# RKlompUU/fhe-regex

Measured on AMD Instinct MI355X. Metric: TFHE gate-bootstraps/sec; end-to-end match time for /abc/ on 256-char content, higher is better.
Workload: dtype u64

## Files before the change

fhe-regex_amd/csrc/capi.cpp:

```cpp
#include <climits>
#include <cstring>
#include <string>
#include <vector>

#include "ctx.h"
#include "rns.h"

using namespace fr;

namespace fr {

static thread_local std::string g_last_error;
void set_last_error(const std::string& m) { g_last_error = m; }

Params params_from_c(const fr_params* c) {
    Params p;
    if (c) {
        p.k = c->k;
        p.N = c->N;
        p.n = c->n;
        p.ks_base_log = c->ks_base_log;
        p.ks_level = c->ks_level;
        p.pbs_base_log = c->pbs_base_log;
        p.pbs_level = c->pbs_level;
        p.ring = c->ring;
        p.lwe_sigma = c->lwe_sigma;
        p.glwe_sigma = c->glwe_sigma;
    }
    validate_params(p);
    return p;
}
void validate_params(const Params& p) {
    if (p.k < 1 || p.k > 4 || p.N < 256 || p.N > 4096 || (p.N & (p.N - 1)) || p.n < 1 || p.n > 1024)
        throw Error(FR_ERR_INVALID, "invalid params");
    if (p.pbs_base_log != 23 || p.pbs_level != 1) throw Error(FR_ERR_INVALID, "only the 2^23 x 1 PBS gadget is supported");
    if (p.ks_base_log < 1 || p.ks_base_log * p.ks_level > 63) throw Error(FR_ERR_INVALID, "invalid keyswitch gadget");
    if (p.ring != FR_RING_RNS && p.ring != FR_RING_FFT) throw Error(FR_ERR_INVALID, "invalid ring");
    if (p.ring == FR_RING_FFT && !((p.k == 1 && p.N == 2048) || (p.k == 2 && p.N == 1024)))
        throw Error(FR_ERR_INVALID, "the FFT ring is built for (k, N) = (1, 2048) and (2, 1024)");
}

}

static Program one_output(std::vector<PGate>&& gates) {
    Program p;
    p.gates = std::move(gates);
    p.outs.push_back(ProgOut{(int32_t)p.gates.size() - 1, 1, 0});
    compute_levels(p);
    return p;
}
static Program prog_cmp_const(VNode::Op op, uint8_t c) {
    const bool sign = op != VNode::EQ;
    return one_output({nibble_test_gate(sign, 0, 0, c & 15), nibble_test_gate(sign, 0, 1, c >> 4), cmp_final_gate(op, 0, 1)});
}

extern "C" {

const char* fr_last_error(void) { return fr::g_last_error.c_str(); }

int fr_default_params(fr_params* out) {
    FR_TRY({
        NEED(out);
        Params p;
        std::memset(out, 0, sizeof *out);
        out->k = p.k;
        out->N = p.N;
        out->n = p.n;
        out->ks_base_log = p.ks_base_log;
        out->ks_level = p.ks_level;
        out->pbs_base_log = p.pbs_base_log;
        out->pbs_level = p.pbs_level;
        out->ring = p.ring;
        out->lwe_sigma = p.lwe_sigma;
        out->glwe_sigma = p.glwe_sigma;
    })
}

int fr_ctx_create(const fr_params* params, int device, fr_ctx** out) {
    FR_TRY({
        NEED(out);
        *out = nullptr;
        auto ctx = std::make_unique<fr_ctx>();
        ctx->p = params_from_c(params);
        if (device >= 0) ctx->dev = std::make_unique<Device>(ctx->p, device);
        *out = ctx.release();
    })
}

int fr_ctx_destroy(fr_ctx* ctx) {
// ... 462 lines not shown
        NEED((content || !len) && tables && any && start_lo <= start_hi && (starts_out || start_lo == start_hi));
        NEED(m >= 1 && m <= NEEDLE_MAX_CHARS);
        plain_needle(MATCH_NEEDLE_CLEAR, content, len, len, m, start_lo, start_hi, nullptr, nullptr, starts_out, any,
                     tables);
    })
}
int fr_plain_scan_clear_bytes(const uint8_t* content, size_t len, const uint8_t* tables, size_t m, size_t start_lo,
                              size_t start_hi, uint8_t* starts_out, int32_t* any) {
    FR_TRY({
        NEED((content || !len) && tables && any && start_lo <= start_hi && (starts_out || start_lo == start_hi));
        NEED(m >= 1 && m <= NEEDLE_MAX_CHARS && start_hi - start_lo <= ((size_t)1 << 24));
        WindowClasses wc = window_classes(content, len, m, start_lo, start_hi);
        pad_window_text(wc, m);
        plain_needle(MATCH_NEEDLE_WINDOWS, wc.text.data(), wc.text.size(), scan_padded(wc.first.size()), m, start_lo,
                     start_hi, nullptr, &wc.cls, starts_out, any, tables);
    })
}
int fr_dev_select_sum(fr_ctx* ctx, const fr_needle* needle, const uint8_t* content, size_t len, const int32_t* terms,
                      const int32_t* n_terms, size_t n_sums, uint64_t* out) {
    FR_TRY({
        NEED(ctx && needle && (content || !len) && terms && n_terms && out);
        Device& dev = ctx->device();
        if (needle->k != ctx->p.k || needle->N != ctx->p.N)
            throw Error(FR_ERR_INVALID, "needle: k, N do not match the context params");
        dev.select_sum_host(needle->dev, content, len, terms, n_terms, n_sums, out);
    })
}
int fr_dev_select_sum_ms(fr_ctx* ctx, double* ms) {
    FR_TRY({
        NEED(ctx && ms);
        *ms = ctx->device().select_sum_ms();
    })
}
int fr_dev_ring_mul(fr_ctx* ctx, const uint64_t* a, const uint64_t* b, size_t count, uint64_t* out) {
    FR_TRY({
        NEED(ctx && a && b && out);
        ctx->device().ring_mul_host(a, b, count, out);
    })
}
int fr_dev_bench_pbs(fr_ctx* ctx, const fr_ct* in, size_t count, int32_t iters, double* br_ms, double* total_ms) {
    FR_TRY({
        NEED(ctx && in && count && iters > 0 && br_ms && total_ms);
        Device& dev = ctx->device();
        if (!ctx->has_sk) throw Error(FR_ERR_NO_KEY, "server key not generated");
        std::vector<DevGate> gates(count);
        for (size_t i = 0; i < count; ++i) {
            const HandleRec& h = ctx->get(in[i]);
            DevGate& d = gates[i];
            std::memset(&d, 0, sizeof d);
            int nin = 0, off = 0;
            const int w[2] = {1, 4};
            for (int b = 0; b < (h.is_bool ? 1 : 2); ++b) {
                if (h.b[b].slot < 0) {
                    off += w[b] * h.b[b].triv;
                    continue;
                }
                d.in_slot[nin] = h.b[b].slot;
                d.in_w[nin] = w[b];
                ++nin;
            }
            d.n_in = nin;
            d.offset = 2 * off;
            lut_eq(d.lut[0], 1);
            d.n_out = 1;
            d.direct = JOB_DIRECT;
        }
        Slots outs(dev, count);
        for (size_t i = 0; i < count; ++i) gates[i].out_slot[0] = outs[i];
        dev.bench_pbs(gates, iters, br_ms, total_ms);
    })
}

uint64_t fr_debug_scalar(int32_t op, uint64_t x, uint64_t y) {
    switch (op) {
        case 0: return rns::crt((uint32_t)(x % rns::P0), (uint32_t)(x % rns::P1));
        case 1: return (uint64_t)(int64_t)rns::decompose((uint32_t)(x % rns::P0), (uint32_t)(x % rns::P1));
        case 2: return rns::to_torus((uint32_t)(x % rns::P0), (uint32_t)(x % rns::P1));
        case 3: return mod_switch(x, (int)y);
        case 4: {
            int32_t d[5];
            ks_decompose<3, 5>(x, d);
            return (uint64_t)(int64_t)d[y % 5];
        }
        default: return 0;
    }
}

int fr_debug_arena_stats(fr_ctx* ctx, uint64_t* slots, uint64_t* free_slots) {
    FR_TRY({
        NEED(ctx && slots && free_slots);
        Device& dev = ctx->device();
        dev.sync();
        *slots = dev.arena_slots();
        *free_slots = dev.arena_free_slots();
    })
}

int fr_debug_handle_count(fr_ctx* ctx, uint64_t* live) {
    FR_TRY({
        NEED(ctx && live);
        *live = ctx->handles.size() - ctx->free_handles.size();
    })
}

int fr_export_bool_device(fr_ctx* ctx, const fr_ct* h, size_t n, uint64_t* dev_dst) {
    FR_TRY({
        NEED(ctx && (h || !n) && (dev_dst || !n));
        Device& dev = ctx->device();
        std::vector<int> slots(n);
        size_t n_triv = 0;
        for (size_t i = 0; i < n; ++i) {
            slots[i] = ctx->get(h[i]).b[0].slot;
            n_triv += slots[i] < 0;
        }
        Slots tmp(dev, n_triv);
        std::vector<uint64_t> lwe((size_t)ctx->p.lwe_len(), 0);
        for (size_t i = 0, t = 0; i < n; ++i) {
            if (slots[i] >= 0) continue;
            lwe.back() = (uint64_t)ctx->get(h[i]).b[0].triv << DELTA_LOG;
            slots[i] = tmp[t++];
            dev.write_slots(&slots[i], 1, lwe.data());
        }
        dev.slots_to_device(slots.data(), n, dev_dst);
    })
}
int fr_export_bool_device_async(fr_ctx* ctx, const fr_ct* h, size_t n, uint64_t* dev_dst) {
    FR_TRY({
        NEED(ctx && (h || !n) && (dev_dst || !n));
        if (n > 16) throw Error(FR_ERR_INVALID, "fr_export_bool_device_async: at most 16 handles");
        std::vector<int> slots(n);
        for (size_t i = 0; i < n; ++i) {
            const HandleRec& r = ctx->get(h[i]);
            if (r.b[0].slot < 0) return fr_export_bool_device(ctx, h, n, dev_dst);
            slots[i] = r.b[0].slot;
        }
        ctx->device().slots_to_device_async(slots.data(), n, dev_dst);
    })
}
int fr_stream(fr_ctx* ctx, void** stream) {
    FR_TRY({
        NEED(ctx && stream);
        *stream = ctx->device().stream();
    })
}
int fr_import_bool_device(fr_ctx* ctx, const uint64_t* dev_src, size_t n, fr_ct* out) {
    FR_TRY({
        NEED(ctx && out && (dev_src || !n));
        Device& dev = ctx->device();
        Slots slots(dev, n);
        dev.device_to_slots(slots.data(), n, dev_src);
        ctx->adopt(std::move(slots), false, out);
    })
}
static int device_timers(fr_ctx* ctx, double DeviceTimers::*ms, uint64_t DeviceTimers::*launches,
                         uint64_t DeviceTimers::*gates, double* br_ms, double* ks_ms, uint64_t* br_launches,
                         uint64_t* br_gates) {
    FR_TRY({
        NEED(ctx);
        Device& dev = ctx->device();
        dev.sync();
        const DeviceTimers& t = dev.timers();
        if (br_ms) *br_ms = t.*ms;
        if (ks_ms) *ks_ms = t.ks_ms;
        if (br_launches) *br_launches = t.*launches;
        if (br_gates) *br_gates = t.*gates;
    })
// ... 34 lines not shown
```

fhe-regex_amd/csrc/fft_br.hip:

```cpp
#include <hip/hip_ext.h>
#include <hip/hip_runtime.h>

#include <cstring>

#include "device_impl.h"
#include "fft.h"
#include "geo.h"

namespace fr {

template <int M, int E>
using FGeo = NttGeo<M, E, 3, fft_layout_variant(ilog2c(M), ilog2c(E))>;
template <int M, int E>
constexpr int FV = fft_layout_variant(ilog2c(M), ilog2c(E));

__device__ __forceinline__ void cfwd(double2& x, double2& y, double2 c) { fft::fwd_bf(x.x, x.y, y.x, y.y, c.x, c.y); }
__device__ __forceinline__ void cinv(double2& u, double2& v, double2 c) { fft::inv_bf(u.x, u.y, v.x, v.y, c.x, c.y); }

template <int M, int E>
constexpr bool fradix4() {
    return E == 4 && FGeo<M, E>::LOG % 2 == 0;
}
template <int M, int E>
struct FTwr {
    static constexpr int COUNT = fradix4<M, E>() ? FGeo<M, E>::NPH * 3 : FGeo<M, E>::LOG * (E / 2);
    double2 v[COUNT];
};
__device__ __forceinline__ double2 fmul_i(double2 c) { return make_double2(-c.y, c.x); }
__device__ __forceinline__ void cinv_r4(double2 (&x)[4], double2 c, double2 ca, double2 cc) {
    fft::inv_r4(x[0].x, x[0].y, x[1].x, x[1].y, x[2].x, x[2].y, x[3].x, x[3].y, c.x, c.y, ca.x, ca.y, cc.x, cc.y);
}
template <class G, int E, int p, bool REV, class F>
__device__ __forceinline__ void for_butterflies(F&& fn) {
#pragma unroll
    for (int i = 0; i < G::s_end(p) - G::s_begin(p); ++i) {
        const int s = REV ? G::s_end(p) - 1 - i : G::s_begin(p) + i;
        const int dm = 1 << (G::LOG - 1 - s - G::lo(p));
#pragma unroll
        for (int m = 0; m < E; ++m) {
            if (m & dm) continue;
            fn(s, m, dm);
        }
    }
}
template <class G, int p>
__device__ __forceinline__ double2 ftw_at(const double2* tw, int b, int s, int m) {
    return (tw + (b >> (G::LOG - s)))[(1 << s) + (G::template moff<p>(m) >> (G::LOG - s))];
}
template <int M, int E, int p>
__device__ __forceinline__ void ftw_r4(const double2* tw, int tl, double2& c, double2& ca) {
    using G = FGeo<M, E>;
    constexpr int s0 = G::s_begin(p), s1 = s0 + 1;
    const int b = G::template base<p>(tl);
    c = ftw_at<G, p>(tw, b, s0, 0);
    ca = ftw_at<G, p>(tw, b, s1, 0);
}

template <int M, int E, int p>
__device__ __forceinline__ void ffwd_phase(double2 (&x)[E], const double2* tw, int tl) {
    using G = FGeo<M, E>;
    const int b = G::template base<p>(tl);
    for_butterflies<G, E, p, false>([&](int s, int m, int dm) { cfwd(x[m], x[m + dm], ftw_at<G, p>(tw, b, s, m)); });
}
template <int M, int E, int p>
__device__ __forceinline__ void finv_phase(double2 (&x)[E], const double2* tw, int tl) {
    using G = FGeo<M, E>;
    const int b = G::template base<p>(tl);
    for_butterflies<G, E, p, true>([&](int s, int m, int dm) { cinv(x[m], x[m + dm], ftw_at<G, p>(tw, b, s, m)); });
}
template <int M, int E, int p>
__device__ __forceinline__ void finv_phase_lds(double2 (&x)[E], const double2* tw, const double2* twc, int tl) {
    if constexpr (fradix4<M, E>()) {
        using G = FGeo<M, E>;
        double2 c, ca;
        ftw_r4<M, E, p>(tw, tl, c, ca);
        const double2 cc = ftw_at<G, p>(twc, G::template base<p>(tl), G::s_begin(p), 0);
        cinv_r4(x, c, ca, cc);
    } else {
        finv_phase<M, E, p>(x, tw, tl);
    }
}

template <int M, int E, int p>
constexpr bool ftw_wave_uniform() {
    using G = FGeo<M, E>;
    for (int w = 0; w * 64 < G::T; ++w)
        for (int s = G::s_begin(p); s < G::s_end(p); ++s) {
            const int ref = geo_base(G::LOG, G::e, p, w * 64, FV<M, E>) >> (G::LOG - s);
            for (int l = 1; l < 64; ++l)
                if ((geo_base(G::LOG, G::e, p, w * 64 + l, FV<M, E>) >> (G::LOG - s)) != ref) return false;
// ... 235 lines not shown
template <int K, int NB, class KeyAt>
__device__ __forceinline__ void key_products(const double (&bre)[2][NB], const double (&bim)[2][NB], int mb, uint32_t ei,
                                             uint32_t ej, uint32_t sm, KeyAt&& key, double& kor, double& koi,
                                             double (&kxr)[K], double (&kxi)[K]) {
    double cr[3], ci[3];
#pragma unroll
    for (int h = 1; h < 3; ++h)
        slot_factor(bre[h - 1][mb], bim[h - 1][mb], h == 1 ? ei : ej, sm, cr[h], ci[h]);
    fft::cmul(cr[1], ci[1], cr[2], ci[2], cr[0], ci[0]);
#pragma unroll
    for (int gg = 0; gg < 3; ++gg) {
        const double c1r = cr[gg] - 1.0, c1i = ci[gg];
        const double2 Bo = key(gg, 0);
        if (gg == 0) fft::cmul(Bo.x, Bo.y, c1r, c1i, kor, koi);
        else fft::cmac(Bo.x, Bo.y, c1r, c1i, kor, koi);
#pragma unroll
        for (int q = 0; q < K; ++q) {
            const double2 Bx = key(gg, 1 + q);
            if (gg == 0) fft::cmul(Bx.x, Bx.y, c1r, c1i, kxr[q], kxi[q]);
            else fft::cmac(Bx.x, Bx.y, c1r, c1i, kxr[q], kxi[q]);
        }
    }
}
constexpr int KEY_AHEAD = -1;
constexpr int KEY_TOP = -2;
constexpr int KEY_NEVER = -3;
struct FbrKeySchedule {
    int g[3];
    constexpr int group_at(int when) const {
        for (int i = 0; i < 3; ++i)
            if (g[i] == when) return i;
        return 3;
    }
    constexpr int ahead() const { return (g[0] == KEY_AHEAD) + (g[1] == KEY_AHEAD) + (g[2] == KEY_AHEAD); }
    constexpr bool ok(int nph) const {
        for (int i = 0; i < 3; ++i) {
            if ((g[i] == KEY_AHEAD) != (i < ahead())) return false;
            if (g[i] != KEY_AHEAD && g[i] != KEY_NEVER && (group_at(g[i]) != i || g[i] >= nph)) return false;
        }
        return true;
    }
};

template <int N_, int K_, int E_, bool LAT_, int B_ = 1, bool KP_ = false>
struct FbrShape {
    static constexpr int N = N_, K = K_, E = E_, B = B_;
    static constexpr bool LAT = LAT_, KP = KP_;
    static constexpr int M = N / 2;
    using G = FGeo<M, E>;
    static_assert(fexchanges_conflict_free<M, E>(), "LDS maps must make every exchange conflict-free");
    static_assert(G::base_matches_geo(), "base<p> must be the index map the LDS-map proofs reason about");
    static_assert(G::key_slot_matches_idx(), "the Fourier key's lane layout is the last-phase layout");
    static_assert(!LAT || E == 4, "the latency shape holds a step's GGSW values in registers: E = 4");
    static_assert(B == 1 || (B == 2 && LAT && K == 1 && E == 4), "pair shape: the k = 1 latency geometry");
    static_assert(!KP || (LAT && B == 1 && K == 1 && E == 4), "key products: the k = 1 latency shape");

    static constexpr int T = M / E;
    static constexpr int NT = (K + 1) * T;
    static constexpr int MIN_WAVES = LAT ? 2 : K == 1 ? (E == 4 ? 4 : 2) : (E == 4 ? 3 : 2);
    static constexpr int TP_GROUPS = K == 1 ? 2 : (E == 8 ? 3 : 2);
    static constexpr int NB = E >= 4 ? E / 4 : 1;
    static constexpr int LAST = G::NPH - 1, XL = G::XL;
    static constexpr int LOG2N2 = G::LOG + 2;
    static constexpr bool TWR = LAT && K == 1;
    static constexpr int BS = (K + 1) * G::NP;
    static constexpr bool PSIQ = !LAT || B > 1;
    static constexpr int NPSI = KP ? 0 : PSIQ ? N / 2 : 2 * N;
    static constexpr int NTWC = fradix4<M, E>() && !TWR ? N / 4 : 0;

    static constexpr FbrKeySchedule KEYS = !LAT || KP ? FbrKeySchedule{{KEY_NEVER, KEY_NEVER, KEY_NEVER}}
                                           : B > 1    ? FbrKeySchedule{{KEY_AHEAD, 2, 4}}
                                           : K == 1   ? FbrKeySchedule{{KEY_AHEAD, KEY_AHEAD, KEY_TOP}}
                                                      : FbrKeySchedule{{KEY_AHEAD, KEY_AHEAD, 3}};
    static constexpr int NPF = KEYS.ahead();
    static_assert(KEYS.ok(G::NPH), "key schedule: ahead groups first, then distinct places that exist");

    struct Lds {
        static constexpr int XBUF = 0;
        static constexpr int IBUF = LAT ? XBUF + B * BS : XBUF;
        static constexpr int TW = IBUF + B * BS;
        static constexpr int PSI = TW + (B == 1 ? M : 0);
        static constexpr int TWC = PSI + NPSI;
        static constexpr size_t LUT = 16 * (size_t)(TWC + NTWC);
        static constexpr size_t ABAR = LUT + B * 16 * MAX_OUT;
        static constexpr size_t ABAR_END = ABAR + B * 2 * 1026;
        static constexpr size_t WTERMS = B == 1 ? ABAR_END : 16 * (size_t)IBUF;
        static constexpr size_t WCNT = WTERMS + 4 * B * 16 * MAX_OUT;
        static constexpr size_t WCNT_END = WCNT + 4 * B * MAX_OUT;
        static constexpr size_t NXT = B == 1 ? WCNT_END : ABAR_END;
        static constexpr size_t BYTES = NXT + 2 * 514;
    };
    static_assert(B == 1 || Lds::WCNT_END <= 16 * (size_t)(Lds::IBUF + B * BS),
                  "pair shape: the terms inside the inverse rows");
    static_assert(Lds::BYTES == 16 * (size_t)((LAT ? 2 : 1) * B * BS + (B == 1 ? M : 0) + NPSI + NTWC) +
                                    B * (16 * MAX_OUT + 2 * 1026) + (B == 1 ? 4 * 17 * MAX_OUT : 0) + 2 * 514,
                  "LDS total: the end of the last region is the sum of the regions");
    static_assert(Lds::BYTES <= (LAT ? 160 * 1024 : 160 * 1024 / TP_GROUPS), "LDS per workgroup of the shape");
};

typedef unsigned int fr_v4u __attribute__((ext_vector_type(4)));
__device__ __forceinline__ __amdgpu_buffer_rsrc_t bsk_rsrc(const double2* bsk) {
    return __builtin_amdgcn_make_buffer_rsrc((void*)bsk, 0, 0x7fffffff, 0x00020000);
}
__device__ __forceinline__ double2 bsk_load(__amdgpu_buffer_rsrc_t r, uint32_t lane_off, uint32_t uoff) {
    const fr_v4u v = __builtin_amdgcn_raw_buffer_load_b128(r, (int)lane_off, (int)uoff, 0);
    double2 d;
    __builtin_memcpy(&d, &v, 16);
    return d;
}

template <int K>
__device__ __forceinline__ int other_row(int P, int q) {
    return q < P ? q : q + 1;
}
template <int K, int M, int T>
__device__ __forceinline__ constexpr uint32_t ggsw_off(int g, int r, int c, int m) {
    constexpr uint32_t GG = (uint32_t)(K + 1) * (K + 1) * M;
    return g * GG + (uint32_t)(r * (K + 1) + c) * M + (uint32_t)m * T;
}
template <int K, int M>
constexpr uint32_t ggsw_step_bytes() {
    return 3u * 16u * (uint32_t)((K + 1) * (K + 1) * M);
}
template <int M, int T, int K>
__device__ __forceinline__ void load_slot(double2 (&B)[3][K + 1], __amdgpu_buffer_rsrc_t rs, uint32_t sbase, int P,
                                          int m, uint32_t lane_off) {
#pragma unroll
    for (int gg = 0; gg < 3; ++gg) {
        B[gg][0] = bsk_load(rs, lane_off, sbase + 16u * ggsw_off<K, M, T>(gg, P, P, m));
#pragma unroll
        for (int q = 0; q < K; ++q)
            B[gg][1 + q] = bsk_load(rs, lane_off, sbase + 16u * ggsw_off<K, M, T>(gg, other_row<K>(P, q), P, m));
    }
}
template <class G>
__device__ __forceinline__ uint32_t leaf_exp(int tl, int m) {
    return (1u + 4u * (__brev((uint32_t)G::template idx<G::NPH - 1>(tl, m)) >> (32 - G::LOG))) &
           (uint32_t)((1 << G::LOG) - 1);
}
__device__ __forceinline__ constexpr uint32_t brv2(int m) { return ((m & 1) << 1) | ((m >> 1) & 1); }

template <int N>
__device__ __forceinline__ uint64_t test_poly(int t, bool direct, const uint8_t* lut0) {
    constexpr int box = N / 16, half = box / 2;
    if (!direct) return 1ULL << (DELTA_LOG - 1);
    const int mm = (t + half) / box;
    return mm < 16 ? (uint64_t)lut0[mm] << DELTA_LOG : (uint64_t)0 - ((uint64_t)lut0[0] << DELTA_LOG);
}
template <int N>
__device__ __forceinline__ uint64_t w_step64(const uint64_t* row, const uint32_t* terms, int nt, int j) {
    uint64_t acc = 0;
    for (int t = 0; t < nt; ++t) {
        const uint32_t tm = terms[t];
        int src = j - (int)(tm & 0xFFFF);
        int64_t d = (int64_t)(tm >> 16) - 128;
        if (src < 0) {
            src += N;
            d = -d;
        }
        acc += (uint64_t)d * row[src];
    }
    return acc;
}

template <int M, int E>
__device__ __forceinline__ void fbr_publish(uint64_t* arow, const double (&alo)[E], const double (&ahi)[E], int tl) {
#pragma unroll
    for (int m = 0; m < E; ++m) {
        const int j = FGeo<M, E>::template idx<0>(tl, m);
        arow[j] = fft::torus_of_acc(alo[m]);
        arow[j + M] = fft::torus_of_acc(ahi[m]);
    }
}
template <int N>
__device__ __forceinline__ void fbr_terms(int tid, int n_out, int kind, const uint8_t* lut, uint32_t* wterms, int* wcnt) {
    if (tid < n_out && kind == JOB_MULTI) wcnt[tid] = lut_terms<N>(lut + 16 * tid, wterms + 16 * tid);
}
template <int N, int K, int NT>
__device__ __forceinline__ void fbr_outputs(int tid, const uint64_t* ab, const DevGate& gate, int n_out, int kind,
                                            const uint32_t* wterms, const int* wcnt, uint64_t* arena, int slot_stride) {
    constexpr int big = K * N;
    if (kind != JOB_MULTI) {
        uint64_t* out = arena + (size_t)gate.out_slot[0] * slot_stride;
        const uint64_t post = kind == JOB_SIGN ? (1ULL << (DELTA_LOG - 1)) : 0;
        for (int c = tid; c <= big; c += NT) {
            const ExtractIdx x = extract_index<N, K>(c);
            const uint64_t v = ab[x.pp * N + x.j];
            out[c] = (x.neg ? (uint64_t)0 - v : v) + (c == big ? post : 0);
        }
        return;
    }
    for (int f = 0; f < n_out; ++f) {
        const uint32_t* tf = wterms + 16 * f;
        const int nt = wcnt[f];
        uint64_t* out = arena + (size_t)gate.out_slot[f] * slot_stride;
        for (int c = tid; c <= big; c += NT) {
            const ExtractIdx x = extract_index<N, K>(c);
            const uint64_t v = w_step64<N>(ab + x.pp * N, tf, nt, x.j);
            out[c] = x.neg ? (uint64_t)0 - v : v;
        }
    }
}

template <int N, int K>
constexpr uint32_t kpre_step_bytes() {
    return 16u * (uint32_t)((K + 1) * (K + 1) * (N / 2));
}

template <int N, int K, int E, bool LAT, int B, bool KP, bool ACC = false>
__device__ __forceinline__ void fbr_rotate(const uint64_t* ks, int ks_stride, int n, const DevGate* gates, int n_gates,
                                           const double2* bsk, const double2* tw_g, const double2* psi_g,
                                           const uint16_t* leaf_g, uint64_t* arena, int slot_stride, const double2* kpre,
                                           const uint64_t* sel = nullptr) {
    using S = FbrShape<N, K, E, LAT, B, KP>;
    using G = typename S::G;
    using L = typename S::Lds;
    static_assert(!(ACC && KP), "selector launches never take the key-products path");
    constexpr int M = S::M, T = S::T, NT = S::NT, NB = S::NB, BS = S::BS, LAST = S::LAST, XL = S::XL;
    constexpr int LOG2N2 = S::LOG2N2, NPSI = S::NPSI, NTWC = S::NTWC, NPF = S::NPF;
    constexpr bool TWR = S::TWR, PSIQ = S::PSIQ;
    extern __shared__ __attribute__((aligned(16))) double2 fsm[];
    uint8_t* const fsb = (uint8_t*)fsm;
    double2 *xbuf = fsm + L::XBUF, *ibuf = fsm + L::IBUF, *tw = fsm + L::TW, *psi = fsm + L::PSI, *twc = fsm + L::TWC;
    uint8_t* lut = fsb + L::LUT;
    uint16_t* abar = (uint16_t*)(fsb + L::ABAR);
    uint32_t* wterms = (uint32_t*)(fsb + L::WTERMS);
    int* wcnt = (int*)(fsb + L::WCNT);
    uint16_t* nxt = (uint16_t*)(fsb + L::NXT);

    const int tid = threadIdx.x;
    const int P = __builtin_amdgcn_readfirstlane(tid / T), tl = tid % T;
    int gb[B];
    bool has[B];
    const uint64_t* in[B];
    int n_out[B], kind[B];
#pragma unroll
    for (int b = 0; b < B; ++b) {
        const int gi = B * (int)blockIdx.x + b;
        has[b] = gi < n_gates;
        gb[b] = has[b] ? gi : B * (int)blockIdx.x;
        in[b] = ks + (size_t)gb[b] * ks_stride;
        n_out[b] = gates[gb[b]].n_out;
        kind[b] = gates[gb[b]].direct;
    }
    if constexpr (B == 1)
        for (int i = tid; i < M; i += NT) tw[i] = tw_g[i];
    for (int i = tid; i < NPSI; i += NT) psi[psi_slot(i)] = psi_g[i];
    for (int i = 1 + tid; i < NTWC; i += NT) {
        const int s0 = 31 - __builtin_clz((unsigned)i), b = i - (1 << s0);
        if (s0 & 1) continue;
        const double2 c = tw_g[i], ca = tw_g[(2 << s0) + 2 * b];
        fft::cmul(c.x, c.y, ca.x, ca.y, twc[i].x, twc[i].y);
    }
    uint32_t bbar[B];
#pragma unroll
    for (int b = 0; b < B; ++b) {
        uint8_t* lb = lut + b * 16 * MAX_OUT;
        uint16_t* ab = abar + b * 1026;
        for (int i = tid; i < 16 * n_out[b]; i += NT) lb[i] = gates[gb[b]].lut[i / 16][i % 16];
        for (int i = tid; i < n; i += NT) ab[i] = (uint16_t)mod_switch(in[b][i], LOG2N2);
        if (tid == 0) ab[n] = 0;
        bbar[b] = mod_switch(in[b][n], LOG2N2);
    }
    uint32_t Lb[NB];
#pragma unroll
    for (int bb = 0; bb < NB; ++bb) Lb[bb] = leaf_exp<G>(tl, 4 * bb);
    __syncthreads();

    double alo[B][E], ahi[B][E];
#pragma unroll
    for (int b = 0; b < B; ++b) {
        if constexpr (ACC) {
            const uint64_t* A = sel + ((size_t)acc_selector(gates[gb[b]]) * (K + 1) + P) * N;
#pragma unroll
            for (int m = 0; m < E; ++m) {
                const int j = G::template idx<0>(tl, m);
                uint64_t v[2];
#pragma unroll
                for (int h = 0; h < 2; ++h) {
                    const int s = (j + h * M + (int)bbar[b]) & (2 * N - 1);
                    const uint64_t tv = A[s & (N - 1)];
                    v[h] = s < N ? tv : (uint64_t)0 - tv;
                }
                alo[b][m] = fft::acc_of_torus(v[0]);
                ahi[b][m] = fft::acc_of_torus(v[1]);
            }
            continue;
        }
        const bool direct = kind[b] == JOB_DIRECT;
#pragma unroll
        for (int m = 0; m < E; ++m) {
            const int j = G::template idx<0>(tl, m);
            uint64_t v[2];
#pragma unroll
            for (int h = 0; h < 2; ++h) {
                const int s = (j + h * M + (int)bbar[b]) & (2 * N - 1);
                const uint64_t tv = test_poly<N>(s & (N - 1), direct, lut + b * 16 * MAX_OUT);
                v[h] = s < N ? tv : (uint64_t)0 - tv;
            }
            alo[b][m] = P == K ? fft::acc_of_torus(v[0]) : 0.0;
            ahi[b][m] = P == K ? fft::acc_of_torus(v[1]) : 0.0;
        }
    }

    double2* row = xbuf + P * G::NP;
    double2* irow = ibuf + P * G::NP;
    const int bl = G::template base<LAST>(tl);
    double2* row_bl = row + G::template at<XL>(bl);
    const double2* orow_bl[K];
#pragma unroll
    for (int q = 0; q < K; ++q) orow_bl[q] = xbuf + other_row<K>(P, q) * G::NP + G::template at<XL>(bl);
    const __amdgpu_buffer_rsrc_t rs = bsk_rsrc(bsk);
    const uint32_t lane_off = 16u * (uint32_t)tl;
    const int steps = (n + 1) / 2;
    double2 gv[3][K + 1][LAT && !KP ? E : 1];
    double2 kv[K + 1][KP ? E : 1];
    FTwr<M, TWR ? E : 2> twr;
    if constexpr (TWR) ftw_load_phase<M, E, 0, (B > 1)>(twr, B == 1 ? tw : tw_g, tl);
#ifdef FR_BR_TIMING
    uint64_t tseg[6] = {0, 0, 0, 0, 0, 0};
    uint64_t tlast = __builtin_amdgcn_s_memtime();
    const uint64_t tstart = tlast;
#endif
    auto load_ggsw = [&](int gg, int tt) {
        if constexpr (!KP) {
            const uint32_t sb = (uint32_t)__builtin_amdgcn_readfirstlane(tt) * ggsw_step_bytes<K, M>();
#pragma unroll
            for (int m = 0; m < E; ++m) {
                gv[gg][0][m] = bsk_load(rs, lane_off, sb + 16u * ggsw_off<K, M, T>(gg, P, P, m));
#pragma unroll
                for (int q = 0; q < K; ++q)
                    gv[gg][1 + q][m] =
                        bsk_load(rs, lane_off, sb + 16u * ggsw_off<K, M, T>(gg, other_row<K>(P, q), P, m));
            }
        }
    };
    const __amdgpu_buffer_rsrc_t rk =
        bsk_rsrc(KP ? kpre + (size_t)blockIdx.x * ((size_t)((n + 1) / 2) * (kpre_step_bytes<N, K>() / 16)) : bsk);
    auto load_kp = [&](int tt) {
        if constexpr (KP) {
            const uint32_t sb = (uint32_t)__builtin_amdgcn_readfirstlane(tt) * kpre_step_bytes<N, K>();
#pragma unroll
            for (int r = 0; r <= K; ++r)
#pragma unroll
                for (int m = 0; m < E; ++m)
                    kv[r][m] = bsk_load(rk, lane_off, sb + 16u * (uint32_t)(((P * (K + 1) + r) * E + m) * T));
        }
    };
    constexpr bool LATPF = NPF > 0;
    auto idle = [&](int t) {
        uint32_t z = 0;
#pragma unroll
        for (int b = 0; b < B; ++b) z |= abar[b * 1026 + 2 * t] | abar[b * 1026 + 2 * t + 1];
        return z == 0;
    };
    if constexpr (LATPF || KP) {
        for (int t = tid; t <= steps; t += NT) {
            int tt = t;
            while (tt < steps && idle(tt)) ++tt;
            nxt[t] = (uint16_t)tt;
        }
        __syncthreads();
        const int t0 = __builtin_amdgcn_readfirstlane((int)nxt[0]);
        for (int gg = 0; gg < NPF; ++gg) load_ggsw(gg, t0 < steps ? t0 : 0);
        load_kp(t0 < steps ? t0 : 0);
    }
    for (int t = 0; t < steps; ++t) {
        if (idle(t)) continue;
        BR_STAMP(0);
        const uint32_t sbase = (uint32_t)__builtin_amdgcn_readfirstlane(t) * ggsw_step_bytes<K, M>();
        constexpr int G_TOP = S::KEYS.group_at(KEY_TOP);
        if constexpr (G_TOP < 3) {
            __builtin_amdgcn_sched_barrier(0);
            load_ggsw(G_TOP, t);
            __builtin_amdgcn_sched_barrier(0);
        }
        uint32_t ei[B], ej[B];
#pragma unroll
        for (int b = 0; b < B; ++b) {
            ei[b] = __builtin_amdgcn_readfirstlane((uint32_t)abar[b * 1026 + 2 * t]);
            ej[b] = __builtin_amdgcn_readfirstlane((uint32_t)abar[b * 1026 + 2 * t + 1]);
        }
        double bre[B][2][NB], bim[B][2][NB];
        auto psi_factors = [&]() {
#pragma unroll
            for (int b = 0; b < B; ++b)
#pragma unroll
                for (int h = 0; h < 2; ++h)
#pragma unroll
                    for (int bb = 0; bb < NB; ++bb)
                        key_psi_base<N, PSIQ>(psi, h == 0 ? ei[b] : ej[b], Lb[bb], bre[b][h][bb], bim[b][h][bb]);
        };
        if constexpr (LAT && B == 1 && !KP) psi_factors();
        double2 x[B][E];
#pragma unroll
        for (int b = 0; b < B; ++b)
#pragma unroll
            for (int m = 0; m < E; ++m)
                x[b][m] = make_double2(fft::acc_digit<23>(alo[b][m]), fft::acc_digit<23>(ahi[b][m]));
        BR_STAMP(1);
        fforward_from<M, E, 0, LAT, TWR, B, BS>(x, row, twr, tw, tl, [&](auto ph) {
            constexpr int g = S::KEYS.group_at(decltype(ph)::value);
            if constexpr (g < 3) {
                __builtin_amdgcn_sched_barrier(0);
                load_ggsw(g, t);
                __builtin_amdgcn_sched_barrier(0);
            }
        });
        BR_STAMP(2);
#pragma unroll
        for (int b = 0; b < B; ++b)
#pragma unroll
            for (int m = 0; m < E; ++m) row_bl[b * BS + G::template at<XL>(G::template moff<LAST>(m))] = x[b][m];
        constexpr bool AHEAD = !LAT && E == 8;
        constexpr bool PRE0 = !LAT;
        double2 Bc[3][K + 1];
        if constexpr (PRE0) load_slot<M, T, K>(Bc, rs, sbase, P, 0, lane_off);
        __syncthreads();
        if constexpr (!LAT || B > 1) psi_factors();
#pragma unroll
        for (int m = 0; m < E; ++m) {
            double2 Bn[3][K + 1];
            if constexpr (AHEAD) {
                if (m + 1 < E) load_slot<M, T, K>(Bn, rs, sbase, P, m + 1, lane_off);
                __builtin_amdgcn_sched_barrier(0);
            } else if constexpr (!LAT) {
                if (!PRE0 || m > 0) load_slot<M, T, K>(Bc, rs, sbase, P, m, lane_off);
            }
#pragma unroll
            for (int b = 0; b < B; ++b) {
                const double2 own = x[b][m];
                double2 oth[K];
#pragma unroll
                for (int q = 0; q < K; ++q) oth[q] = orow_bl[q][b * BS + G::template at<XL>(G::template moff<LAST>(m))];
                double kor, koi, kxr[K], kxi[K];
                if constexpr (KP) {
                    kor = kv[0][m].x, koi = kv[0][m].y;
#pragma unroll
                    for (int q = 0; q < K; ++q) kxr[q] = kv[1 + q][m].x, kxi[q] = kv[1 + q][m].y;
                } else {
                    const uint32_t sm = brv2(m);
                    auto key_at = [&](int gg, int r) __attribute__((always_inline)) {
                        return LAT ? gv[gg][r][LAT ? m : 0] : Bc[gg][r];
                    };
                    key_products<K>(bre[b], bim[b], m >> 2, ei[b], ej[b], sm, key_at, kor, koi, kxr, kxi);
                }
                double zr, zi;
                fft::cmul(own.x, own.y, kor, koi, zr, zi);
#pragma unroll
                for (int q = 0; q < K; ++q) fft::cmac(oth[q].x, oth[q].y, kxr[q], kxi[q], zr, zi);
                x[b][m] = make_double2(zr, zi);
            }
            if constexpr (!LAT) {
                __builtin_amdgcn_sched_barrier(0);
            }
            if constexpr (AHEAD) {
#pragma unroll
                for (int gg = 0; gg < 3; ++gg)
#pragma unroll
                    for (int r = 0; r <= K; ++r) Bc[gg][r] = Bn[gg][r];
            }
        }
        if constexpr (LATPF || KP) {
            const int tn = __builtin_amdgcn_readfirstlane((int)nxt[t + 1]);
            __builtin_amdgcn_sched_barrier(0);
            for (int gg = 0; gg < NPF; ++gg) load_ggsw(gg, tn < steps ? tn : t);
            load_kp(tn < steps ? tn : t);
            __builtin_amdgcn_sched_barrier(0);
        }
        BR_STAMP(3);
        finverse_from<M, E, LAST, LAT, TWR, B, BS>(x, irow, twr, tw, twc, tl);
        BR_STAMP(4);
#pragma unroll
        for (int b = 0; b < B; ++b)
#pragma unroll
            for (int m = 0; m < E; ++m) {
                alo[b][m] = fft::acc_reduce<23>(alo[b][m] + x[b][m].x);
                ahi[b][m] = fft::acc_reduce<23>(ahi[b][m] + x[b][m].y);
            }
        BR_STAMP(5);
    }
#ifdef FR_BR_TIMING
    if (blockIdx.x == 0 && tid == 0)
        printf("FBR_TIMING E=%d LAT=%d steps=%d total=%lu digits=%lu fwd=%lu mac=%lu inv=%lu acc=%lu top=%lu\n", E, (int)LAT,
               steps, (unsigned long)(__builtin_amdgcn_s_memtime() - tstart), (unsigned long)tseg[1],
               (unsigned long)tseg[2], (unsigned long)tseg[3], (unsigned long)tseg[4], (unsigned long)tseg[5],
               (unsigned long)tseg[0]);
#endif

    __syncthreads();
    uint64_t* accs = (uint64_t*)xbuf;
    static_assert(B == 1 || 8 * B * (K + 1) * N <= 16 * B * BS, "pair shape: u64 rows inside the forward rows");
#pragma unroll
    for (int b = 0; b < B; ++b) {
        fbr_publish<M, E>(accs + (b * (K + 1) + P) * N, alo[b], ahi[b], tl);
        fbr_terms<N>(tid, n_out[b], kind[b], lut + b * 16 * MAX_OUT, wterms + b * 16 * MAX_OUT, wcnt + b * MAX_OUT);
    }
    __syncthreads();
#pragma unroll
    for (int b = 0; b < B; ++b)
        if (has[b])
            fbr_outputs<N, K, NT>(tid, accs + b * (K + 1) * N, gates[gb[b]], n_out[b], kind[b], wterms + b * 16 * MAX_OUT,
                                  wcnt + b * MAX_OUT, arena, slot_stride);
}

template <int N, int K, int E, bool LAT, int B = 1>
__global__ void __launch_bounds__((FbrShape<N, K, E, LAT, B>::NT), (FbrShape<N, K, E, LAT, B>::MIN_WAVES))
k_blind_rotate_fft(const uint64_t* __restrict__ ks, int ks_stride, int n, const DevGate* __restrict__ gates,
                   int n_gates, const double2* __restrict__ bsk, const double2* __restrict__ tw_g,
                   const double2* __restrict__ psi_g, const uint16_t* __restrict__ leaf_g, uint64_t* __restrict__ arena,
                   int slot_stride) {
    fbr_rotate<N, K, E, LAT, B, false>(ks, ks_stride, n, gates, n_gates, bsk, tw_g, psi_g, leaf_g, arena, slot_stride,
                                       nullptr);
}
template <int N, int K, int E, bool LAT, int B = 1>
__global__ void __launch_bounds__((FbrShape<N, K, E, LAT, B>::NT), (FbrShape<N, K, E, LAT, B>::MIN_WAVES))
k_blind_rotate_fft_kp(const uint64_t* __restrict__ ks, int ks_stride, int n, const DevGate* __restrict__ gates,
                      int n_gates, const double2* __restrict__ tw_g, uint64_t* __restrict__ arena, int slot_stride,
                      const double2* __restrict__ kpre) {
    fbr_rotate<N, K, E, LAT, B, true>(ks, ks_stride, n, gates, n_gates, nullptr, tw_g, nullptr, nullptr, arena,
                                      slot_stride, kpre);
}

template <int N, int K, int E, bool LAT, int B = 1>
__global__ void __launch_bounds__((FbrShape<N, K, E, LAT, B>::NT), (FbrShape<N, K, E, LAT, B>::MIN_WAVES))
k_blind_rotate_fft_acc(const uint64_t* __restrict__ ks, int ks_stride, int n, const DevGate* __restrict__ gates,
                       int n_gates, const double2* __restrict__ bsk, const double2* __restrict__ tw_g,
                       const double2* __restrict__ psi_g, const uint16_t* __restrict__ leaf_g,
                       uint64_t* __restrict__ arena, int slot_stride, const uint64_t* __restrict__ sel) {
    fbr_rotate<N, K, E, LAT, B, false, true>(ks, ks_stride, n, gates, n_gates, bsk, tw_g, psi_g, leaf_g, arena,
                                             slot_stride, nullptr, sel);
}

template <int N>
__global__ void __launch_bounds__((FbrShape<N, 1, 4, true>::T))
k_key_products(const uint64_t* __restrict__ ks, int ks_stride, int n, int n_gates, const double2* __restrict__ bsk,
               const double2* __restrict__ psi_g, double2* __restrict__ kpre) {
    using S = FbrShape<N, 1, 4, true>;
    using G = typename S::G;
    constexpr int K = S::K, E = S::E, M = S::M, T = S::T, LOG2N2 = S::LOG2N2;
    constexpr uint32_t GG = (uint32_t)(K + 1) * (K + 1) * M;
    __shared__ __attribute__((aligned(16))) double2 psi[N / 2];
    const int tl = threadIdx.x, t = (int)blockIdx.x, P = (int)blockIdx.y;
    const int steps = (n + 1) / 2;
    for (int i = tl; i < N / 2; i += T) psi[psi_slot(i)] = psi_g[i];
    const __amdgpu_buffer_rsrc_t rs = bsk_rsrc(bsk);
    const uint32_t lane_off = 16u * (uint32_t)tl, sb = (uint32_t)t * ggsw_step_bytes<K, M>();
    double2 gv[3][K + 1][E];
#pragma unroll
    for (int gg = 0; gg < 3; ++gg)
// ... 349 lines not shown
```

Before: 126,700.

## Compact live blind-rotation steps into a packed schedule walked without idle checks

```diff
diff --git a/fhe-regex_amd/csrc/capi.cpp b/fhe-regex_amd/csrc/capi.cpp
--- a/fhe-regex_amd/csrc/capi.cpp
+++ b/fhe-regex_amd/csrc/capi.cpp
@@ -5,6 +5,7 @@
 
 #include "ctx.h"
 #include "rns.h"
+#include "step_sched.h"
 
 using namespace fr;
 
@@ -633,6 +634,8 @@
             ks_decompose<3, 5>(x, d);
             return (uint64_t)(int64_t)d[y % 5];
         }
+        case 5: return step_sched::put(x, (int)((y >> step_sched::FIELD_BITS) % step_sched::FIELDS), (uint32_t)y);
+        case 6: return step_sched::get(x, (int)(y % step_sched::FIELDS));
         default: return 0;
     }
 }
diff --git a/fhe-regex_amd/csrc/fft_br.hip b/fhe-regex_amd/csrc/fft_br.hip
--- a/fhe-regex_amd/csrc/fft_br.hip
+++ b/fhe-regex_amd/csrc/fft_br.hip
@@ -6,6 +6,7 @@
 #include "device_impl.h"
 #include "fft.h"
 #include "geo.h"
+#include "step_sched.h"
 
 namespace fr {
 
@@ -407,18 +408,23 @@
         static constexpr int PSI = TW + (B == 1 ? M : 0);
         static constexpr int TWC = PSI + NPSI;
         static constexpr size_t LUT = 16 * (size_t)(TWC + NTWC);
-        static constexpr size_t ABAR = LUT + B * 16 * MAX_OUT;
+        static constexpr size_t LIVE = LUT + B * 16 * MAX_OUT;
+        static constexpr size_t SCHED = LIVE + (LAT ? 8 * (step_sched::MAX_STEPS / 64) : 0);
+        static constexpr size_t SCHED_END = SCHED + (LAT ? 8 * (step_sched::MAX_STEPS + 1) : 0);
+        static constexpr size_t ABAR = B == 1 ? SCHED_END : 16 * (size_t)IBUF;
         static constexpr size_t ABAR_END = ABAR + B * 2 * 1026;
         static constexpr size_t WTERMS = B == 1 ? ABAR_END : 16 * (size_t)IBUF;
         static constexpr size_t WCNT = WTERMS + 4 * B * 16 * MAX_OUT;
         static constexpr size_t WCNT_END = WCNT + 4 * B * MAX_OUT;
-        static constexpr size_t NXT = B == 1 ? WCNT_END : ABAR_END;
-        static constexpr size_t BYTES = NXT + 2 * 514;
+        static constexpr size_t BYTES = B == 1 ? WCNT_END : SCHED_END;
     };
-    static_assert(B == 1 || Lds::WCNT_END <= 16 * (size_t)(Lds::IBUF + B * BS),
-                  "pair shape: the terms inside the inverse rows");
-    static_assert(Lds::BYTES == 16 * (size_t)((LAT ? 2 : 1) * B * BS + (B == 1 ? M : 0) + NPSI + NTWC) +
-                                    B * (16 * MAX_OUT + 2 * 1026) + (B == 1 ? 4 * 17 * MAX_OUT : 0) + 2 * 514,
+    static_assert(B == 1 || (Lds::WCNT_END <= 16 * (size_t)(Lds::IBUF + B * BS) &&
+                             Lds::ABAR_END <= 16 * (size_t)(Lds::IBUF + B * BS)),
+                  "pair shape: abar (prologue) and the terms (tail) inside the inverse rows");
+    static_assert(Lds::LIVE % 8 == 0 && Lds::ABAR % 4 == 0 && Lds::WTERMS % 4 == 0, "u64 / u32 regions aligned");
+    static_assert(Lds::BYTES == 16 * (size_t)((LAT ? 2 : 1) * B * BS + (B == 1 ? M : 0) + NPSI + NTWC) + B * 16 * MAX_OUT +
+                                    (LAT ? 8 * (step_sched::MAX_STEPS / 64 + step_sched::MAX_STEPS + 1) : 0) +
+                                    (B == 1 ? 2 * 1026 + 4 * 17 * MAX_OUT : 0),
                   "LDS total: the end of the last region is the sum of the regions");
     static_assert(Lds::BYTES <= (LAT ? 160 * 1024 : 160 * 1024 / TP_GROUPS), "LDS per workgroup of the shape");
 };
@@ -551,7 +557,8 @@
     uint16_t* abar = (uint16_t*)(fsb + L::ABAR);
     uint32_t* wterms = (uint32_t*)(fsb + L::WTERMS);
     int* wcnt = (int*)(fsb + L::WCNT);
-    uint16_t* nxt = (uint16_t*)(fsb + L::NXT);
+    uint64_t* live = (uint64_t*)(fsb + L::LIVE);
+    uint64_t* sched = (uint64_t*)(fsb + L::SCHED);
 
     const int tid = threadIdx.x;
     const int P = __builtin_amdgcn_readfirstlane(tid / T), tl = tid % T;
@@ -673,13 +680,44 @@
         }
     };
     constexpr bool LATPF = NPF > 0;
+    constexpr bool WALK = LAT && K == 1;
+    static_assert(LAT == (LATPF || KP), "every latency shape prefetches the next unskipped step");
+    static_assert(!KP || WALK, "key products: addressed by the schedule's step index, first loaded after its build");
+    uint16_t* nxt = (uint16_t*)sched;
+    static_assert(2 * (step_sched::MAX_STEPS + 2) <= 8 * (step_sched::MAX_STEPS + 1), "nxt inside the schedule's region");
+    auto sched_entry = [&](int i) {
+        const uint64_t v = sched[i];
+        const uint32_t lo = (uint32_t)__builtin_amdgcn_readfirstlane((uint32_t)v);
+        const uint32_t hi = (uint32_t)__builtin_amdgcn_readfirstlane((uint32_t)(v >> 32));
+        return ((uint64_t)hi << 32) | lo;
+    };
     auto idle = [&](int t) {
         uint32_t z = 0;
 #pragma unroll
         for (int b = 0; b < B; ++b) z |= abar[b * 1026 + 2 * t] | abar[b * 1026 + 2 * t + 1];
         return z == 0;
     };
-    if constexpr (LATPF || KP) {
+    uint64_t ent = step_sched::END_ENTRY;
+    int si = 0;
+    if constexpr (WALK) {
+        static_assert(NT % 64 == 0, "whole waves: a wave's ballot covers 64 consecutive steps");
+        for (int t0 = 0; t0 < steps; t0 += NT) {
+            const int t = t0 + tid;
+            const uint64_t m = __ballot(t < steps && !idle(t));
+            if ((tid & 63) == 0 && t < steps) live[t >> 6] = m;
+        }
+        __syncthreads();
+        for (int t = tid; t <= steps; t += NT) {
+            const int rank = step_sched::rank_below(live, t);
+            if (t == steps) sched[rank] = step_sched::END_ENTRY;
+            else if (!idle(t)) sched[rank] = step_sched::entry_of<B>(abar, 1026, t);
+        }
+        __syncthreads();
+        ent = sched_entry(0);
+        const int t0 = (int)step_sched::step(ent);
+        for (int gg = 0; gg < NPF; ++gg) load_ggsw(gg, t0 != (int)step_sched::END ? t0 : 0);
+        load_kp(t0 != (int)step_sched::END ? t0 : 0);
+    } else if constexpr (LATPF) {
         for (int t = tid; t <= steps; t += NT) {
             int tt = t;
             while (tt < steps && idle(tt)) ++tt;
@@ -688,10 +726,12 @@
         __syncthreads();
         const int t0 = __builtin_amdgcn_readfirstlane((int)nxt[0]);
         for (int gg = 0; gg < NPF; ++gg) load_ggsw(gg, t0 < steps ? t0 : 0);
-        load_kp(t0 < steps ? t0 : 0);
-    }
-    for (int t = 0; t < steps; ++t) {
-        if (idle(t)) continue;
+    }
+    auto step_from = [&](int t) { return WALK ? (int)step_sched::step(ent) : t; };
+    auto more = [&](int t) { return WALK ? t != (int)step_sched::END : t < steps; };
+    for (int t = step_from(0); more(t); t = step_from(t + 1)) {
+        if constexpr (!WALK)
+            if (idle(t)) continue;
         BR_STAMP(0);
         const uint32_t sbase = (uint32_t)__builtin_amdgcn_readfirstlane(t) * ggsw_step_bytes<K, M>();
         constexpr int G_TOP = S::KEYS.group_at(KEY_TOP);
@@ -703,8 +743,13 @@
         uint32_t ei[B], ej[B];
 #pragma unroll
         for (int b = 0; b < B; ++b) {
-            ei[b] = __builtin_amdgcn_readfirstlane((uint32_t)abar[b * 1026 + 2 * t]);
-            ej[b] = __builtin_amdgcn_readfirstlane((uint32_t)abar[b * 1026 + 2 * t + 1]);
+            if constexpr (WALK) {
+                ei[b] = step_sched::pair_i(ent, b);
+                ej[b] = step_sched::pair_j(ent, b);
+            } else {
+                ei[b] = __builtin_amdgcn_readfirstlane((uint32_t)abar[b * 1026 + 2 * t]);
+                ej[b] = __builtin_amdgcn_readfirstlane((uint32_t)abar[b * 1026 + 2 * t + 1]);
+            }
         }
         double bre[B][2][NB], bim[B][2][NB];
         auto psi_factors = [&]() {
@@ -786,11 +831,18 @@
                     for (int r = 0; r <= K; ++r) Bc[gg][r] = Bn[gg][r];
             }
         }
-        if constexpr (LATPF || KP) {
+        if constexpr (LATPF && !WALK) {
             const int tn = __builtin_amdgcn_readfirstlane((int)nxt[t + 1]);
             __builtin_amdgcn_sched_barrier(0);
             for (int gg = 0; gg < NPF; ++gg) load_ggsw(gg, tn < steps ? tn : t);
-            load_kp(tn < steps ? tn : t);
+            __builtin_amdgcn_sched_barrier(0);
+        }
+        if constexpr (WALK) {
+            ent = sched_entry(++si);
+            const int tn = (int)step_sched::step(ent);
+            __builtin_amdgcn_sched_barrier(0);
+            for (int gg = 0; gg < NPF; ++gg) load_ggsw(gg, tn != (int)step_sched::END ? tn : t);
+            load_kp(tn != (int)step_sched::END ? tn : t);
             __builtin_amdgcn_sched_barrier(0);
         }
         BR_STAMP(3);
diff --git a/fhe-regex_amd/csrc/step_sched.h b/fhe-regex_amd/csrc/step_sched.h
--- /dev/null
+++ b/fhe-regex_amd/csrc/step_sched.h
@@ -0,0 +1,49 @@
+#pragma once
+#include "common.h"
+
+namespace fr {
+namespace step_sched {
+
+constexpr int FIELD_BITS = 12, FIELDS = 5;
+constexpr uint32_t FIELD_MASK = (1u << FIELD_BITS) - 1;
+constexpr uint32_t END = FIELD_MASK;
+constexpr int MAX_STEPS = 512;
+static_assert(FIELDS * FIELD_BITS <= 64 && MAX_STEPS <= (int)END, "five fields in 64 bits, END above every step");
+
+FR_HD constexpr uint64_t put(uint64_t e, int f, uint32_t v) {
+    return e | ((uint64_t)(v & FIELD_MASK) << (FIELD_BITS * f));
+}
+FR_HD constexpr uint32_t get(uint64_t e, int f) {
+    const uint32_t lo = (uint32_t)e, hi = (uint32_t)(e >> 32);
+    const int s = FIELD_BITS * f;
+    return (s + FIELD_BITS <= 32 ? lo >> s : s >= 32 ? hi >> (s - 32) : (lo >> s) | (hi << (32 - s))) & FIELD_MASK;
+}
+FR_HD constexpr uint32_t step(uint64_t e) { return get(e, 0); }
+FR_HD constexpr uint32_t pair_i(uint64_t e, int b) { return get(e, 1 + 2 * b); }
+FR_HD constexpr uint32_t pair_j(uint64_t e, int b) { return get(e, 2 + 2 * b); }
+constexpr uint64_t END_ENTRY = END;
+
+FR_HD int rank_below(const uint64_t* live, int t) {
+    int rank = 0;
+    for (int w = 0; w < (t >> 6); ++w) rank += __builtin_popcountll(live[w]);
+    const uint64_t mine = (t & 63) ? live[t >> 6] : 0;
+    return rank + __builtin_popcountll(mine & ((1ULL << (t & 63)) - 1));
+}
+template <int B>
+FR_HD uint64_t entry_of(const uint16_t* abar, int stride, int t) {
+    static_assert(1 + 2 * B <= FIELDS, "the step and B pairs in one entry");
+    uint64_t e = put(0, 0, (uint32_t)t);
+FR_UNROLL
+    for (int b = 0; b < B; ++b) {
+        e = put(e, 1 + 2 * b, abar[b * stride + 2 * t]);
+        e = put(e, 2 + 2 * b, abar[b * stride + 2 * t + 1]);
+    }
+    return e;
+}
+
+static_assert(step(put(put(put(0, 0, 370), 1, 4095), 2, 0)) == 370 && pair_i(put(put(0, 0, 370), 1, 4095), 0) == 4095 &&
+                  pair_j(put(put(put(put(0, 0, 0), 3, 4095), 4, 4095), 2, 1), 1) == 4095,
+              "fields do not overlap");
+
+}
+}
```

Result: faster. 130,400 (median of 6 runs) (+3.0%).
